# menyifang/MIMO

Measured on NVIDIA H100. Metric: frames/sec @ 512x512x24f, 20 DDIM steps, higher is better.
Workload: dtype fp16

## Files before the change

include/mimo_b200.h:

```cpp
#ifndef MIMO_B200_H_
#define MIMO_B200_H_

#include <stdint.h>

#ifdef __cplusplus
extern "C" {
#endif

#define MIMO_OK 0
#define MIMO_ERR_ARG (-1)
#define MIMO_ERR_CUDA (-2)
#define MIMO_ERR_DEVICE (-3)

#define MIMO_F16 0
#define MIMO_BF16 1

#define MIMO_ACT_NONE 0
#define MIMO_ACT_SILU 1
#define MIMO_ACT_GEGLU 2

const char* mimo_version(void);
const char* mimo_last_error(void);
int mimo_device_check(int dev);
int mimo_abi_sizeof(int which);

typedef struct {
  const void* bias;
  const void* rowvec;
  int64_t rows_per_group;
  int64_t ld_rowvec;
  const void* residual;
  int64_t ld_res;
  float scale;
  int act;
} mimo_epilogue;

typedef struct {
  const void* a;
  int64_t lda;
  const void* a1;
  int64_t lda1;
  const void* w;
  int64_t ldw;
  void* out;
  int64_t ldo;
  int32_t M, N, K;
  int32_t K1;
  int32_t dtype;
  mimo_epilogue ep;
  void* workspace;
  int64_t workspace_bytes;
} mimo_gemm_params;
int mimo_gemm(const mimo_gemm_params* p, void* stream);
int mimo_gemm_geglu_granule(int32_t N);

typedef struct {
  const void* a;
  int64_t lda;
  const float* a_scale;
  const void* w;
  int64_t ldw;
  const float* w_scale;
  void* out;
  int64_t ldo;
  int32_t M, N, K;
  int32_t dtype;
  mimo_epilogue ep;
  void* workspace;
  int64_t workspace_bytes;
} mimo_gemm_e4m3_params;
int mimo_gemm_e4m3(const mimo_gemm_e4m3_params* p, void* stream);

typedef struct {
  const void* x0;
  int32_t c0;
  const void* x1;
  int32_t c1;
  const void* w;
  void* out;
  int64_t ldo;
  int32_t n, h, w_, cout;
  int32_t dtype;
  mimo_epilogue ep;
  void* workspace;
  int64_t workspace_bytes;
} mimo_conv3x3_params;
int mimo_conv3x3(const mimo_conv3x3_params* p, void* stream);
int mimo_conv_up2x(const mimo_conv3x3_params* p, void* stream);

int mimo_im2col3x3(const void* x, void* col, int32_t n, int32_t h, int32_t w, int32_t c, int32_t stride,
                   int32_t upshift, int32_t pad_lo, int64_t ldcol, int32_t dtype, void* stream);

typedef struct {
  const void* x0;
  int32_t c0;
  const void* x1;
  int32_t c1;
  const void* gamma;
  const void* beta;
  void* out;
  float* stats;
  int32_t n, hw, groups;
  float eps;
  int32_t silu;
  int32_t dtype;
} mimo_groupnorm_params;
int mimo_groupnorm(const mimo_groupnorm_params* p, void* stream);
int64_t mimo_groupnorm_workspace_bytes(const mimo_groupnorm_params* p);

typedef struct {
  const void* x0;
  int32_t c0;
  const void* x1;
  int32_t c1;
  const void* gamma;
  const void* beta;
  void* out;
  float* table;
  int64_t table_bytes;
  float* stats;
  int32_t samples, frames, table_frames, hw, groups;
  float eps;
  int32_t silu;
  int32_t dtype;
} mimo_groupnorm_window_params;
int mimo_groupnorm_window(const mimo_groupnorm_window_params* p, void* stream);
int mimo_groupnorm_window_partials(const mimo_groupnorm_window_params* p, void* stream);
int mimo_groupnorm_window_apply(const mimo_groupnorm_window_params* p, void* stream);
int64_t mimo_groupnorm_window_table_bytes(const mimo_groupnorm_window_params* p);

int mimo_layernorm(const void* x, const void* gamma, const void* beta, void* out, int64_t rows, int32_t c,
                   float eps, const void* pe, int64_t rows_per_frame, int32_t frames, int32_t pe_frame_offset,
                   int32_t dtype, void* stream);
int mimo_layernorm_e4m3(const void* x, const void* gamma, const void* beta, void* out, float* scale, int64_t rows,
                        int32_t c, float eps, const void* pe, int64_t rows_per_frame, int32_t frames,
                        int32_t pe_frame_offset, int32_t dtype, void* stream);

typedef struct {
  const void* q;
  const void* k;
  const void* v;
  int64_t ld_qkv;
  const void* bank_k;
  const void* bank_v;
  int64_t ld_bank;
  int32_t lb;
  int32_t nb;
  const int32_t* bank_index;
  void* out;
  int64_t ld_out;
  int32_t n, lq, heads, d;
  float scale;
  int32_t dtype;
} mimo_attn_params;
int mimo_attn_spatial(const mimo_attn_params* p, void* stream);

typedef struct {
  const void* q;
  int64_t ld_q;
  const void* k;
  const void* v;
  int64_t ld_kv;
  void* out;
  int64_t ld_out;
  int64_t chunk_stride_rows;
  int32_t batch, q_frames, kv_frames, frames_per_chunk;
  int32_t hw, heads, d;
  float scale;
  int32_t dtype;
} mimo_attn_temporal_params;
int mimo_attn_temporal(const mimo_attn_temporal_params* p, void* stream);

#define MIMO_MAX_PEERS 8
typedef struct {
  const void* peer_src[MIMO_MAX_PEERS];
  void* peer_ready[MIMO_MAX_PEERS];
  void* ctl;
  void* dst;
  const void* residual;
  int32_t mode, G, r;
  int32_t b, fl, hw, C;
  int32_t dtype;
  int32_t max_blocks;
  int32_t timeout_ms;
} mimo_exchange_params;
int mimo_exchange(const mimo_exchange_params* p, void* stream);
int mimo_peer_alloc(int64_t bytes, void** ptr, void* handle64);
int mimo_peer_open(const void* handle64, void** ptr);
int mimo_peer_close(void* ptr);
int mimo_peer_free(void* ptr);

int mimo_ncfhw_to_nhwc(const void* src, void* dst, int32_t b, int32_t c, int32_t f, int32_t h, int32_t w,
                       int32_t cpad, int32_t src_is_f32, int32_t dtype, void* stream);
int mimo_nhwc_to_ncfhw(const void* src, void* dst, int32_t b, int32_t c, int32_t f, int32_t h, int32_t w,
                       int32_t ld, int32_t dst_is_f32, int32_t dtype, void* stream);
int mimo_upsample2x(const void* x, void* out, int32_t n, int32_t h, int32_t w, int32_t c, int32_t dtype, void* stream);
int mimo_upsample_nearest(const void* x, void* out, int32_t n, int32_t h, int32_t w, int32_t oh, int32_t ow, int32_t c,
                          int32_t dtype, void* stream);
int mimo_softmax_rows(void* x, int64_t rows, int32_t cols, int64_t ld, int32_t dtype, void* stream);
int mimo_add(const void* a, const void* b, void* out, int64_t count, int32_t dtype, void* stream);
int mimo_silu(const void* x, void* out, int64_t count, int32_t dtype, void* stream);

int mimo_quick_gelu(const void* x, void* out, int64_t count, int32_t dtype, void* stream);

int mimo_composite_frame(const void* canvas, const void* bk, const float* mask, const void* occ, const void* vid,
                         const void* prev, double factor, void* out, int64_t pixels, void* stream);
// ... 36 lines not shown
```

mimo_b200/csrc/gemm_wgmma.cu:

```cuda
#include <cuda_runtime.h>

#include <cudaTypedefs.h>

#include "../../include/mimo_b200.h"
#include "host_util.h"
#include "ptx.cuh"
#include "wgmma.cuh"

namespace mimo {

constexpr int BM = 128;
constexpr int BK = 64;
constexpr int kGemmThreads = 320;
constexpr int kChunk = 8192;

struct EpiArgs {
  const void* bias;
  const void* rowvec;
  long long rows_per_group;
  long long ld_rowvec;
  float scale;
  int act;
  float* partial;
};

struct ConvGeom {
  int conv;
  int H, W, NI;
  int TW, TH, TN;
  int tiles_w, tiles_h;
  int ctot;
  int c0;
  int kb0, kb1;
  int a_bytes;
  int chunk_bytes;
  int splits;
  int kb_split;
  int ntaps;
  signed char tdx[9], tdy[9];
};

template <int BN, bool kRes, bool kE4m3 = false>
struct GemmCfg {
  static constexpr int kStageBytes = BM * BK * 2 + BN * BK * 2;
  static constexpr int kNChunk = BN / 32;
  static constexpr int kOutBytes = 2 * kChunk;
  static constexpr int kResSlots = kRes ? 2 : 0;
  static constexpr int kResBytes = kResSlots * kChunk;
  static constexpr int kBarBytes = 512;
  static constexpr int kFixed = kBarBytes + 2048  + (kE4m3 ? 3072  : 0) + kOutBytes + kResBytes;
  static constexpr int kMaxStages = (BN >= 256) ? 4 : (BN >= 160 ? 5 : (BN >= 128 ? 6 : 8));
  static constexpr int kFit = (227 * 1024 - kFixed) / kStageBytes;
  static constexpr int kStages = kFit < kMaxStages ? kFit : kMaxStages;
  static constexpr int kSmemBytes = kStages * kStageBytes + kFixed;
  static_assert(kStages >= 3, "pipeline too shallow");
};

template <int BN, bool kBf16, bool kRes>
__global__ void __launch_bounds__(kGemmThreads, 1)
gemm_wgmma_kernel(const __grid_constant__ CUtensorMap tmA0, const __grid_constant__ CUtensorMap tmA1,
                  const __grid_constant__ CUtensorMap tmB, const __grid_constant__ CUtensorMap tmOut,
                  const __grid_constant__ CUtensorMap tmRes, int M, int N, int num_m_tiles, int num_n_tiles,
                  int num_k_blocks, ConvGeom g, EpiArgs ep) {
  constexpr bool kE4m3 = false;
  constexpr const float* a_scale = nullptr;
  constexpr const float* w_scale = nullptr;
#include "gemm_wgmma_body.cuh"
}

template <int BN, bool kBf16, bool kRes>
__global__ void __launch_bounds__(kGemmThreads, 1)
gemm_e4m3_kernel(const __grid_constant__ CUtensorMap tmA0, const __grid_constant__ CUtensorMap tmA1,
                 const __grid_constant__ CUtensorMap tmB, const __grid_constant__ CUtensorMap tmOut,
                 const __grid_constant__ CUtensorMap tmRes, int M, int N, int num_m_tiles, int num_n_tiles,
                 int num_k_blocks, ConvGeom g, EpiArgs ep, const float* __restrict__ a_scale,
                 const float* __restrict__ w_scale) {
  constexpr bool kE4m3 = true;
#include "gemm_wgmma_body.cuh"
}


template <bool kBf16>
__global__ void __launch_bounds__(256)
splitk_reduce_kernel(const float* __restrict__ part, int splits, long long M, int N, const void* __restrict__ bias,
                     const void* __restrict__ rowvec, long long rpg, long long ld_rowvec,
                     const void* __restrict__ res, long long ld_res, float scale, int act, void* __restrict__ out,
                     long long ldo) {
  using C = Cvt<kBf16>;
  using T = typename C::T;
  pdl_launch_dependents();
  pdl_wait();
  const int nv = N >> 3;
  const long long idx = blockIdx.x * static_cast<long long>(blockDim.x) + threadIdx.x;
  if (idx >= M * nv) return;
  const long long row = idx / nv;
  const int col = static_cast<int>(idx - row * nv) * 8;
  float a[8] = {0.f, 0.f, 0.f, 0.f, 0.f, 0.f, 0.f, 0.f};
  for (int s = 0; s < splits; ++s) {
    const float4* p = reinterpret_cast<const float4*>(part + (static_cast<long long>(s) * M + row) * N + col);
    const float4 u0 = p[0], u1 = p[1];
    a[0] += u0.x, a[1] += u0.y, a[2] += u0.z, a[3] += u0.w;
    a[4] += u1.x, a[5] += u1.y, a[6] += u1.z, a[7] += u1.w;
  }
  float cst[8] = {0.f, 0.f, 0.f, 0.f, 0.f, 0.f, 0.f, 0.f};
  auto add_vec = [&](const T* v, float* dst, bool scaled_fma) {
    const uint4 b = *reinterpret_cast<const uint4*>(v);
    const uint32_t w[4] = {b.x, b.y, b.z, b.w};
#pragma unroll
    for (int j = 0; j < 4; ++j) {
      const float2 t = C::unpack(w[j]);
      if (scaled_fma) {
        dst[2 * j] = fmaf(t.x, scale, dst[2 * j]);
        dst[2 * j + 1] = fmaf(t.y, scale, dst[2 * j + 1]);
      } else {
        dst[2 * j] += t.x;
        dst[2 * j + 1] += t.y;
      }
    }
  };
  if (bias) add_vec(static_cast<const T*>(bias) + col, cst, false);
  if (rowvec) add_vec(static_cast<const T*>(rowvec) + (row / rpg) * ld_rowvec + col, cst, false);
  float f[8];
#pragma unroll
  for (int j = 0; j < 8; ++j) f[j] = fmaf(a[j], scale, cst[j] * scale);
  if (res) add_vec(static_cast<const T*>(res) + row * ld_res + col, f, true);
  if (act == MIMO_ACT_SILU) {
#pragma unroll
    for (int j = 0; j < 8; ++j) f[j] = silu_f(f[j]);
  }
  uint4 o;
  o.x = C::pack(f[0], f[1]);
  o.y = C::pack(f[2], f[3]);
  o.z = C::pack(f[4], f[5]);
  o.w = C::pack(f[6], f[7]);
  *reinterpret_cast<uint4*>(static_cast<T*>(out) + row * ldo + col) = o;
}

static int pick_splits(long long tiles, int nkb, long long M, int N, int64_t ws_bytes) {
  if (tiles * 2 > num_sms() || nkb < 32) return 1;
  long long s = num_sms() / tiles;
  if (s > nkb / 16) s = nkb / 16;
  if (s > 16) s = 16;
  while (s > 1 && s * M * N * 4 > ws_bytes) --s;
  return s < 2 ? 1 : static_cast<int>(s);
}

struct Maps {
  CUtensorMap a0, a1, b, out, res;
};

template <int BN, bool kBf16, bool kRes>
static int launch_cfg(const Maps& m, int M, int N, int mt, int nt, int nkb, const ConvGeom& g, const EpiArgs& ep,
                      cudaStream_t st) {
  using Cfg = GemmCfg<BN, kRes>;
  auto kern = gemm_wgmma_kernel<BN, kBf16, kRes>;
  static bool attr_done = false;
  if (!attr_done) {
    cudaError_t e = cudaFuncSetAttribute(kern, cudaFuncAttributeMaxDynamicSharedMemorySize, Cfg::kSmemBytes);
    if (e != cudaSuccess) return set_cuda_error("cudaFuncSetAttribute(gemm)", e);
    attr_done = true;
  }
  const int tiles = mt * nt;
  const int grid = tiles < num_sms() ? tiles : num_sms();
  cudaError_t e = launch_k(kern, dim3(grid), dim3(kGemmThreads), Cfg::kSmemBytes, st, m.a0, m.a1, m.b, m.out, m.res, M, N, mt,
                           nt, nkb, g, ep);
  if (e == cudaSuccess) e = cudaGetLastError();
  if (e != cudaSuccess) return set_cuda_error("gemm launch", e);
  return MIMO_OK;
}

template <bool kBf16>
static int launch_bn(int bn, bool res, const Maps& m, int M, int N, int mt, int nt, int nkb, const ConvGeom& g,
                     const EpiArgs& ep, cudaStream_t st) {
  switch (bn) {
    case 64:
      return res ? launch_cfg<64, kBf16, true>(m, M, N, mt, nt, nkb, g, ep, st)
                 : launch_cfg<64, kBf16, false>(m, M, N, mt, nt, nkb, g, ep, st);
    case 128:
      return res ? launch_cfg<128, kBf16, true>(m, M, N, mt, nt, nkb, g, ep, st)
                 : launch_cfg<128, kBf16, false>(m, M, N, mt, nt, nkb, g, ep, st);
    case 160:
      return res ? launch_cfg<160, kBf16, true>(m, M, N, mt, nt, nkb, g, ep, st)
                 : launch_cfg<160, kBf16, false>(m, M, N, mt, nt, nkb, g, ep, st);
    case 192:
      return res ? launch_cfg<192, kBf16, true>(m, M, N, mt, nt, nkb, g, ep, st)
                 : launch_cfg<192, kBf16, false>(m, M, N, mt, nt, nkb, g, ep, st);
    case 256:
      return res ? launch_cfg<256, kBf16, true>(m, M, N, mt, nt, nkb, g, ep, st)
                 : launch_cfg<256, kBf16, false>(m, M, N, mt, nt, nkb, g, ep, st);
  }
  return set_error(MIMO_ERR_ARG, "gemm: unsupported BN");
}

int pick_bn(int N, bool geglu, long long m_tiles);

template <bool kBf16>
static int launch_e4m3(int bn, bool res, const Maps& m, int M, int N, int mt, int nt, int nkb, const ConvGeom& g,
                       const EpiArgs& ep, const float* a_scale, const float* w_scale, cudaStream_t st) {
  auto run = [&](auto kern, int smem) -> int {
    static bool attr_done[2][2][2] = {};
    bool& done = attr_done[bn == 256][kBf16][res];
    if (!done) {
      cudaError_t e = cudaFuncSetAttribute(kern, cudaFuncAttributeMaxDynamicSharedMemorySize, smem);
      if (e != cudaSuccess) return set_cuda_error("cudaFuncSetAttribute(gemm_e4m3)", e);
      done = true;
    }
    const int tiles = mt * nt;
    const int grid = tiles < num_sms() ? tiles : num_sms();
    cudaError_t e = launch_k(kern, dim3(grid), dim3(kGemmThreads), smem, st, m.a0, m.a1, m.b, m.out, m.res, M, N, mt, nt,
                             nkb, g, ep, a_scale, w_scale);
    if (e == cudaSuccess) e = cudaGetLastError();
    if (e != cudaSuccess) return set_cuda_error("gemm_e4m3 launch", e);
    return MIMO_OK;
  };
  if (bn == 192)
    return res ? run(gemm_e4m3_kernel<192, kBf16, true>, GemmCfg<192, true, true>::kSmemBytes)
               : run(gemm_e4m3_kernel<192, kBf16, false>, GemmCfg<192, false, true>::kSmemBytes);
  if (bn == 256)
    return res ? run(gemm_e4m3_kernel<256, kBf16, true>, GemmCfg<256, true, true>::kSmemBytes)
               : run(gemm_e4m3_kernel<256, kBf16, false>, GemmCfg<256, false, true>::kSmemBytes);
  return set_error(MIMO_ERR_ARG, "mimo_gemm_e4m3: unsupported BN");
}

static int pick_bn_e4m3(int N, bool geglu) {
  if (geglu) return pick_bn(N, true, 1 << 20);
  const int pad256 = (N + 255) / 256 * 256 - N, pad192 = (N + 191) / 192 * 192 - N;
  return pad192 < pad256 ? 192 : 256;
}

static int g_force_bn = 0;

int pick_bn(int N, bool geglu, long long m_tiles) {
  if (g_force_bn) return g_force_bn;
  if (geglu) {
    if (N % 256 == 0) return 256;
    if (N % 128 == 0) return 128;
    return 64;
  }
  const int cands[5] = {256, 192, 160, 128, 64};
  int best = 64;
  double best_eff = -1.0;
  for (int i = 0; i < 5; ++i) {
    const int bn = cands[i];
    const int nt = (N + bn - 1) / bn;
    double eff = static_cast<double>(N) / (static_cast<double>(nt) * bn);
    const long long tiles = m_tiles * nt;
    if (tiles < num_sms() && bn > 64) eff *= 0.5 + 0.5 * static_cast<double>(tiles) / num_sms();
    if (eff > best_eff + 1e-9) {
      best_eff = eff;
      best = bn;
    }
  }
  return best;
}

static EpiArgs make_epi(const mimo_epilogue& e, int N) {
  EpiArgs a;
  a.bias = e.bias;
  a.rowvec = e.rowvec;
  a.rows_per_group = e.rows_per_group > 0 ? e.rows_per_group : 1;
  if (a.rows_per_group > 0x7fffffffLL) a.rows_per_group = 0x7fffffffLL;
  a.ld_rowvec = e.ld_rowvec > 0 ? e.ld_rowvec : N;
  a.scale = e.scale;
  a.act = e.act;
  a.partial = nullptr;
  return a;
}

static int g_splitk = 0;

static int launch_reduce(int dtype, const float* part, int splits, long long M, int N, const mimo_epilogue& e, void* out,
                         long long ldo, cudaStream_t st) {
  const long long total = M * (N / 8);
  const unsigned blocks = div_up(total, 256);
  const long long rpg = e.rows_per_group > 0 ? e.rows_per_group : 1;
  const long long ldr = e.ld_rowvec > 0 ? e.ld_rowvec : N;
  cudaError_t err = dtype == MIMO_BF16
                        ? launch_k(splitk_reduce_kernel<true>, dim3(blocks), dim3(256), 0, st, part, splits, M, N, e.bias,
                                   e.rowvec, rpg, ldr, e.residual, static_cast<long long>(e.ld_res), e.scale, e.act, out, ldo)
                        : launch_k(splitk_reduce_kernel<false>, dim3(blocks), dim3(256), 0, st, part, splits, M, N, e.bias,
                                   e.rowvec, rpg, ldr, e.residual, static_cast<long long>(e.ld_res), e.scale, e.act, out, ldo);
  if (err == cudaSuccess) err = cudaGetLastError();
  if (err != cudaSuccess) return set_cuda_error("split-K reduce launch", err);
  return MIMO_OK;
}

}

using namespace mimo;

extern "C" int mimo_debug_splitk(int mode) {
  g_splitk = mode;
  return 0;
}

extern "C" int mimo_debug_force_bn(int bn) {
  g_force_bn = bn;
  return 0;
}

extern "C" int mimo_gemm_geglu_granule(int32_t N) { return pick_bn(N, true, 1 << 20) / 2; }

extern "C" int mimo_gemm(const mimo_gemm_params* p, void* stream) {
  if (!p || !p->a || !p->w || !p->out) return set_error(MIMO_ERR_ARG, "mimo_gemm: null pointer");
  if (p->M <= 0 || p->N <= 0 || p->K <= 0) return set_error(MIMO_ERR_ARG, "mimo_gemm: empty problem");
  if ((p->K % 8) || (p->lda % 8) || (p->ldw % 8) || (p->N % 8) || (p->ldo % 8))
    return set_error(MIMO_ERR_ARG, "mimo_gemm: K, N, lda, ldw, ldo must be multiples of 8");
  if (p->ep.residual && (p->ep.ld_res % 8)) return set_error(MIMO_ERR_ARG, "mimo_gemm: ld_res % 8 != 0");
  const bool geglu = p->ep.act == MIMO_ACT_GEGLU;
  if (geglu && (p->ep.residual || p->ep.rowvec))
    return set_error(MIMO_ERR_ARG, "mimo_gemm: GEGLU takes neither a residual nor a row vector");
  if (int rc = ensure_device()) return rc;
  const int mt = (p->M + BM - 1) / BM;
  const int K1 = p->a1 ? p->K1 : 0;
  if (K1 < 0 || (K1 % 8) || (p->a1 && (p->lda1 % 8))) return set_error(MIMO_ERR_ARG, "mimo_gemm: K1/lda1 % 8 != 0");
  const int kb0 = (p->K + BK - 1) / BK;
  const int kb1 = (K1 + BK - 1) / BK;
  const int nkb = kb0 + kb1;
  int bn = pick_bn(p->N, geglu, mt);
  int splits = 1;
  if (!geglu && g_splitk && p->workspace && !g_force_bn) {
    const int bn_wide = pick_bn(p->N, false, 1 << 20);
    splits = pick_splits(static_cast<long long>(mt) * ((p->N + bn_wide - 1) / bn_wide), nkb, p->M, p->N, p->workspace_bytes);
    if (splits > 1) bn = bn_wide;
  }
  if (geglu && (p->N % bn)) return set_error(MIMO_ERR_ARG, "mimo_gemm: GEGLU needs N % tile == 0");
  const int nt = (p->N + bn - 1) / bn;
  const bool res = p->ep.residual != nullptr && !geglu && splits == 1;

  Maps m;
  const uint64_t adim[2] = {static_cast<uint64_t>(p->K), static_cast<uint64_t>(p->M)};
  const uint64_t astr[1] = {static_cast<uint64_t>(p->lda) * 2};
  const uint32_t abox[2] = {BK, BM};
  if (int rc = encode_tmap(&m.a0, p->dtype, 2, p->a, adim, astr, abox)) return rc;
  m.a1 = m.a0;
  if (K1) {
    const uint64_t a1dim[2] = {static_cast<uint64_t>(K1), static_cast<uint64_t>(p->M)};
    const uint64_t a1str[1] = {static_cast<uint64_t>(p->lda1) * 2};
    if (int rc = encode_tmap(&m.a1, p->dtype, 2, p->a1, a1dim, a1str, abox)) return rc;
  }
  const uint64_t bdim[2] = {static_cast<uint64_t>(p->K + K1), static_cast<uint64_t>(p->N)};
  const uint64_t bstr[1] = {static_cast<uint64_t>(p->ldw) * 2};
  const uint32_t bbox[2] = {BK, static_cast<uint32_t>(bn)};
  if (int rc = encode_tmap(&m.b, p->dtype, 2, p->w, bdim, bstr, bbox)) return rc;
  const int n_out = geglu ? p->N / 2 : p->N;
  const uint64_t odim[2] = {static_cast<uint64_t>(n_out), static_cast<uint64_t>(p->M)};
  const uint64_t ostr[1] = {static_cast<uint64_t>(p->ldo) * 2};
  const uint32_t obox[2] = {32, BM};
  if (int rc = encode_tmap(&m.out, p->dtype, 2, p->out, odim, ostr, obox, 64)) return rc;
  m.res = m.out;
  if (res) {
    const uint64_t rstr[1] = {static_cast<uint64_t>(p->ep.ld_res) * 2};
    if (int rc = encode_tmap(&m.res, p->dtype, 2, p->ep.residual, odim, rstr, obox, 64)) return rc;
  }

  ConvGeom g = {};
  g.kb0 = kb0;
  g.kb1 = kb1;
  g.c0 = p->K;
  g.chunk_bytes = kChunk;
  g.splits = splits;
  g.kb_split = (nkb + splits - 1) / splits;
  EpiArgs ep = make_epi(p->ep, p->N);
  cudaStream_t st = static_cast<cudaStream_t>(stream);
  if (splits > 1) {
    ep.bias = ep.rowvec = nullptr;
    ep.act = MIMO_ACT_NONE;
    ep.scale = 1.0f;
    ep.partial = static_cast<float*>(p->workspace);
  }
  const int rc = p->dtype == MIMO_BF16 ? launch_bn<true>(bn, res, m, p->M, p->N, mt, nt, nkb, g, ep, st)
                                       : launch_bn<false>(bn, res, m, p->M, p->N, mt, nt, nkb, g, ep, st);
  if (rc || splits == 1) return rc;
  return launch_reduce(p->dtype, ep.partial, splits, p->M, p->N, p->ep, p->out, p->ldo, st);
}

extern "C" int mimo_gemm_e4m3(const mimo_gemm_e4m3_params* p, void* stream) {
  if (!p || !p->a || !p->w || !p->out || !p->a_scale || !p->w_scale)
    return set_error(MIMO_ERR_ARG, "mimo_gemm_e4m3: null pointer");
  if (p->M <= 0 || p->N <= 0 || p->K <= 0) return set_error(MIMO_ERR_ARG, "mimo_gemm_e4m3: empty problem");
  if ((p->K % 16) || (p->lda % 16) || (p->ldw % 16))
    return set_error(MIMO_ERR_ARG, "mimo_gemm_e4m3: K, lda, ldw must be multiples of 16");
  if ((p->N % 8) || (p->ldo % 8)) return set_error(MIMO_ERR_ARG, "mimo_gemm_e4m3: N, ldo must be multiples of 8");
  if ((reinterpret_cast<uintptr_t>(p->a) | reinterpret_cast<uintptr_t>(p->w) | reinterpret_cast<uintptr_t>(p->out) |
       reinterpret_cast<uintptr_t>(p->ep.residual)) % 16)
    return set_error(MIMO_ERR_ARG, "mimo_gemm_e4m3: a, w, out, residual must be 16-byte aligned");
  if (p->ep.residual && (p->ep.ld_res % 8)) return set_error(MIMO_ERR_ARG, "mimo_gemm_e4m3: ld_res % 8 != 0");
  if (p->workspace || p->workspace_bytes) return set_error(MIMO_ERR_ARG, "mimo_gemm_e4m3: split-K is not supported");
  const bool geglu = p->ep.act == MIMO_ACT_GEGLU;
  if (geglu && (p->ep.residual || p->ep.rowvec))
    return set_error(MIMO_ERR_ARG, "mimo_gemm_e4m3: GEGLU takes neither a residual nor a row vector");
  const int bn = pick_bn_e4m3(p->N, geglu);
  if (geglu && (p->N % bn)) return set_error(MIMO_ERR_ARG, "mimo_gemm_e4m3: GEGLU needs N % tile == 0");
  if (bn != 192 && bn != 256) return set_error(MIMO_ERR_ARG, "mimo_gemm_e4m3: GEGLU needs N % 256 == 0");
  if (int rc = ensure_device()) return rc;
  const int mt = (p->M + BM - 1) / BM;
  const int nt = (p->N + bn - 1) / bn;
  const int nkb = (p->K + 2 * BK - 1) / (2 * BK);
  const bool res = p->ep.residual != nullptr && !geglu;

  Maps m;
  const uint64_t adim[2] = {static_cast<uint64_t>(p->K), static_cast<uint64_t>(p->M)};
  const uint64_t astr[1] = {static_cast<uint64_t>(p->lda)};
  const uint32_t abox[2] = {2 * BK, BM};
  if (int rc = encode_tmap(&m.a0, kTmapU8, 2, p->a, adim, astr, abox)) return rc;
  m.a1 = m.a0;
  const uint64_t bdim[2] = {static_cast<uint64_t>(p->K), static_cast<uint64_t>(p->N)};
  const uint64_t bstr[1] = {static_cast<uint64_t>(p->ldw)};
  const uint32_t bbox[2] = {2 * BK, static_cast<uint32_t>(bn)};
  if (int rc = encode_tmap(&m.b, kTmapU8, 2, p->w, bdim, bstr, bbox)) return rc;
  const int n_out = geglu ? p->N / 2 : p->N;
  const uint64_t odim[2] = {static_cast<uint64_t>(n_out), static_cast<uint64_t>(p->M)};
  const uint64_t ostr[1] = {static_cast<uint64_t>(p->ldo) * 2};
  const uint32_t obox[2] = {32, BM};
  if (int rc = encode_tmap(&m.out, p->dtype, 2, p->out, odim, ostr, obox, 64)) return rc;
  m.res = m.out;
  if (res) {
    const uint64_t rstr[1] = {static_cast<uint64_t>(p->ep.ld_res) * 2};
    if (int rc = encode_tmap(&m.res, p->dtype, 2, p->ep.residual, odim, rstr, obox, 64)) return rc;
  }
  ConvGeom g = {};
  g.kb0 = nkb;
  g.c0 = p->K;
  g.chunk_bytes = kChunk;
  g.splits = 1;
  g.kb_split = nkb;
  const EpiArgs ep = make_epi(p->ep, p->N);
  cudaStream_t st = static_cast<cudaStream_t>(stream);
  return p->dtype == MIMO_BF16 ? launch_e4m3<true>(bn, res, m, p->M, p->N, mt, nt, nkb, g, ep, p->a_scale, p->w_scale, st)
                               : launch_e4m3<false>(bn, res, m, p->M, p->N, mt, nt, nkb, g, ep, p->a_scale, p->w_scale, st);
}

static int conv_launch(const mimo_conv3x3_params* p, const void* w, int ntaps, const signed char* tdx,
                       const signed char* tdy, void* out, int sx, int sy, int ow, int oh, void* stream) {
  const int c1 = p->x1 ? p->c1 : 0;
  ConvGeom g = {};
  g.conv = 1;
  g.H = p->h;
  g.W = p->w_;
  g.NI = p->n;
  g.TW = p->w_ < BM ? p->w_ : BM;
  g.TH = BM / g.TW;
  if (g.TH > p->h) g.TH = p->h;
  if (g.TH < 1) g.TH = 1;
  g.TN = BM / (g.TW * g.TH);
  if (g.TN > p->n) g.TN = p->n;
  if (g.TN < 1) g.TN = 1;
  if (g.TN > 1 && g.TH != p->h) g.TN = 1;
  g.tiles_w = (p->w_ + g.TW - 1) / g.TW;
  g.tiles_h = (p->h + g.TH - 1) / g.TH;
  const int tiles_n = (p->n + g.TN - 1) / g.TN;
  g.ctot = p->c0 + c1;
  g.c0 = p->c0;
  g.kb0 = (p->c0 + BK - 1) / BK;
  g.kb1 = (c1 + BK - 1) / BK;
  g.a_bytes = g.TW * g.TH * g.TN * BK * 2;
  g.chunk_bytes = g.TW * g.TH * g.TN * 64;
  g.ntaps = ntaps;
  for (int t = 0; t < 9; ++t) {
    g.tdx[t] = t < ntaps ? tdx[t] : 0;
    g.tdy[t] = t < ntaps ? tdy[t] : 0;
  }
  const int mt = g.tiles_w * g.tiles_h * tiles_n;
  const int nkb = ntaps * (g.kb0 + g.kb1);
  const long long Mrows = static_cast<long long>(p->n) * p->h * p->w_;
  if (Mrows > 0x7fffffffLL) return set_error(MIMO_ERR_ARG, "mimo_conv: too many pixels");
  int bn = pick_bn(p->cout, false, mt);
  int splits = 1;
  if (g_splitk && p->workspace && !g_force_bn && sx == 1 && sy == 1 && p->ldo == p->cout) {
    const int bn_wide = pick_bn(p->cout, false, 1 << 20);
    splits = pick_splits(static_cast<long long>(mt) * ((p->cout + bn_wide - 1) / bn_wide), nkb, Mrows, p->cout,
                         p->workspace_bytes);
    if (splits > 1) bn = bn_wide;
  }
  g.splits = splits;
  g.kb_split = (nkb + splits - 1) / splits;
  const int nt = (p->cout + bn - 1) / bn;
  const bool res = p->ep.residual != nullptr && splits == 1;

  Maps m;
  auto nhwc_map = [&](CUtensorMap* tm, const void* base, int c, long long pitch, uint32_t box_c, int swz, int px,
                      int py, int iw, int ih) {
    const uint64_t dim[4] = {static_cast<uint64_t>(c), static_cast<uint64_t>(p->w_), static_cast<uint64_t>(p->h),
                             static_cast<uint64_t>(p->n)};
    const uint64_t str[3] = {static_cast<uint64_t>(px) * pitch * 2, static_cast<uint64_t>(py) * iw * pitch * 2,
                             static_cast<uint64_t>(ih) * iw * pitch * 2};
    const uint32_t box[4] = {box_c, static_cast<uint32_t>(g.TW), static_cast<uint32_t>(g.TH),
                             static_cast<uint32_t>(g.TN)};
    return encode_tmap(tm, p->dtype, 4, base, dim, str, box, swz);
  };
  if (int rc = nhwc_map(&m.a0, p->x0, p->c0, p->c0, BK, 128, 1, 1, p->w_, p->h)) return rc;
  m.a1 = m.a0;
  if (c1)
    if (int rc = nhwc_map(&m.a1, p->x1, c1, c1, BK, 128, 1, 1, p->w_, p->h)) return rc;
  {
    const uint64_t dim[2] = {static_cast<uint64_t>(ntaps) * g.ctot, static_cast<uint64_t>(p->cout)};
    const uint64_t str[1] = {static_cast<uint64_t>(ntaps) * g.ctot * 2};
    const uint32_t box[2] = {BK, static_cast<uint32_t>(bn)};
    if (int rc = encode_tmap(&m.b, p->dtype, 2, w, dim, str, box)) return rc;
  }
  if (int rc = nhwc_map(&m.out, out, p->cout, p->ldo, 32, 64, sx, sy, ow, oh)) return rc;
  m.res = m.out;
  if (res)
    if (int rc = nhwc_map(&m.res, p->ep.residual, p->cout, p->ep.ld_res, 32, 64, 1, 1, p->w_, p->h)) return rc;

  EpiArgs ep = make_epi(p->ep, p->cout);
  cudaStream_t st = static_cast<cudaStream_t>(stream);
  if (splits > 1) {
    ep.bias = ep.rowvec = nullptr;
    ep.act = MIMO_ACT_NONE;
    ep.scale = 1.0f;
    ep.partial = static_cast<float*>(p->workspace);
  }
  const int rc = p->dtype == MIMO_BF16
                     ? launch_bn<true>(bn, res, m, static_cast<int>(Mrows), p->cout, mt, nt, nkb, g, ep, st)
                     : launch_bn<false>(bn, res, m, static_cast<int>(Mrows), p->cout, mt, nt, nkb, g, ep, st);
  if (rc || splits == 1) return rc;
// ... 41 lines not shown
```

mimo_b200/lib.py:

```python
from __future__ import annotations

import ctypes as C
import os
from pathlib import Path

_PKG = Path(__file__).resolve().parent
LIB_PATH = _PKG / "libmimo_b200.so"

F16, BF16 = 0, 1
ACT_NONE, ACT_SILU, ACT_GEGLU = 0, 1, 2


class MimoError(RuntimeError):
    pass


class Epilogue(C.Structure):
    _fields_ = [
        ("bias", C.c_void_p),
        ("rowvec", C.c_void_p),
        ("rows_per_group", C.c_int64),
        ("ld_rowvec", C.c_int64),
        ("residual", C.c_void_p),
        ("ld_res", C.c_int64),
        ("scale", C.c_float),
        ("act", C.c_int),
    ]


class GemmParams(C.Structure):
    _fields_ = [
        ("a", C.c_void_p), ("lda", C.c_int64),
        ("a1", C.c_void_p), ("lda1", C.c_int64),
        ("w", C.c_void_p), ("ldw", C.c_int64),
        ("out", C.c_void_p), ("ldo", C.c_int64),
        ("M", C.c_int32), ("N", C.c_int32), ("K", C.c_int32), ("K1", C.c_int32),
        ("dtype", C.c_int32),
        ("ep", Epilogue),
        ("workspace", C.c_void_p), ("workspace_bytes", C.c_int64),
    ]


class GemmE4m3Params(C.Structure):
    _fields_ = [
        ("a", C.c_void_p), ("lda", C.c_int64), ("a_scale", C.c_void_p),
        ("w", C.c_void_p), ("ldw", C.c_int64), ("w_scale", C.c_void_p),
        ("out", C.c_void_p), ("ldo", C.c_int64),
        ("M", C.c_int32), ("N", C.c_int32), ("K", C.c_int32),
        ("dtype", C.c_int32),
        ("ep", Epilogue),
        ("workspace", C.c_void_p), ("workspace_bytes", C.c_int64),
    ]


class Conv3x3Params(C.Structure):
    _fields_ = [
        ("x0", C.c_void_p), ("c0", C.c_int32),
        ("x1", C.c_void_p), ("c1", C.c_int32),
        ("w", C.c_void_p),
        ("out", C.c_void_p), ("ldo", C.c_int64),
        ("n", C.c_int32), ("h", C.c_int32), ("w_", C.c_int32), ("cout", C.c_int32),
        ("dtype", C.c_int32),
        ("ep", Epilogue),
        ("workspace", C.c_void_p), ("workspace_bytes", C.c_int64),
    ]


class GroupNormParams(C.Structure):
    _fields_ = [
        ("x0", C.c_void_p), ("c0", C.c_int32),
        ("x1", C.c_void_p), ("c1", C.c_int32),
        ("gamma", C.c_void_p), ("beta", C.c_void_p),
        ("out", C.c_void_p),
        ("stats", C.c_void_p),
        ("n", C.c_int32), ("hw", C.c_int32), ("groups", C.c_int32),
        ("eps", C.c_float),
        ("silu", C.c_int32),
        ("dtype", C.c_int32),
    ]


class GroupNormWindowParams(C.Structure):
    _fields_ = [
        ("x0", C.c_void_p), ("c0", C.c_int32),
        ("x1", C.c_void_p), ("c1", C.c_int32),
        ("gamma", C.c_void_p), ("beta", C.c_void_p),
        ("out", C.c_void_p),
        ("table", C.c_void_p), ("table_bytes", C.c_int64),
        ("stats", C.c_void_p),
        ("samples", C.c_int32), ("frames", C.c_int32), ("table_frames", C.c_int32), ("hw", C.c_int32),
        ("groups", C.c_int32),
        ("eps", C.c_float),
        ("silu", C.c_int32),
        ("dtype", C.c_int32),
    ]


class AttnParams(C.Structure):
    _fields_ = [
        ("q", C.c_void_p), ("k", C.c_void_p), ("v", C.c_void_p), ("ld_qkv", C.c_int64),
        ("bank_k", C.c_void_p), ("bank_v", C.c_void_p), ("ld_bank", C.c_int64),
        ("lb", C.c_int32), ("nb", C.c_int32),
        ("bank_index", C.c_void_p),
        ("out", C.c_void_p), ("ld_out", C.c_int64),
        ("n", C.c_int32), ("lq", C.c_int32), ("heads", C.c_int32), ("d", C.c_int32),
        ("scale", C.c_float),
        ("dtype", C.c_int32),
    ]


class AttnTemporalParams(C.Structure):
    _fields_ = [
        ("q", C.c_void_p), ("ld_q", C.c_int64),
        ("k", C.c_void_p), ("v", C.c_void_p), ("ld_kv", C.c_int64),
        ("out", C.c_void_p), ("ld_out", C.c_int64),
        ("chunk_stride_rows", C.c_int64),
        ("batch", C.c_int32), ("q_frames", C.c_int32), ("kv_frames", C.c_int32), ("frames_per_chunk", C.c_int32),
        ("hw", C.c_int32), ("heads", C.c_int32), ("d", C.c_int32),
        ("scale", C.c_float),
        ("dtype", C.c_int32),
    ]


MAX_PEERS = 8


class ExchangeParams(C.Structure):
    _fields_ = [
        ("peer_src", C.c_void_p * MAX_PEERS), ("peer_ready", C.c_void_p * MAX_PEERS),
        ("ctl", C.c_void_p), ("dst", C.c_void_p), ("residual", C.c_void_p),
        ("mode", C.c_int32), ("G", C.c_int32), ("r", C.c_int32),
        ("b", C.c_int32), ("fl", C.c_int32), ("hw", C.c_int32), ("C", C.c_int32),
        ("dtype", C.c_int32), ("max_blocks", C.c_int32), ("timeout_ms", C.c_int32),
    ]


class CfgMultistepParams(C.Structure):
    _fields_ = [
        ("pred_uncond", C.c_void_p), ("pred_cond", C.c_void_p), ("counter", C.c_void_p), ("frame_stride", C.c_int64),
        ("latents", C.c_void_p), ("count", C.c_int64),
        ("hist_out", C.c_void_p), ("h1", C.c_void_p), ("h2", C.c_void_p), ("noise", C.c_void_p),
        ("guidance", C.c_float), ("a", C.c_float), ("b", C.c_float),
        ("c_x", C.c_float), ("c_m", C.c_float), ("c_1", C.c_float), ("c_2", C.c_float), ("c_n", C.c_float),
        ("dtype", C.c_int32),
    ]


_VP, _I32, _I64, _F = C.c_void_p, C.c_int32, C.c_int64, C.c_float
SYMBOLS = {
    "mimo_version": (C.c_char_p, []),
    "mimo_last_error": (C.c_char_p, []),
    "mimo_device_check": (C.c_int, [C.c_int]),
    "mimo_abi_sizeof": (C.c_int, [C.c_int]),
    "mimo_gemm": (C.c_int, [C.POINTER(GemmParams), _VP]),
    "mimo_gemm_geglu_granule": (C.c_int, [_I32]),
    "mimo_gemm_e4m3": (C.c_int, [C.POINTER(GemmE4m3Params), _VP]),
    "mimo_conv3x3": (C.c_int, [C.POINTER(Conv3x3Params), _VP]),
    "mimo_conv_up2x": (C.c_int, [C.POINTER(Conv3x3Params), _VP]),
    "mimo_im2col3x3": (C.c_int, [_VP, _VP, _I32, _I32, _I32, _I32, _I32, _I32, _I32, _I64, _I32, _VP]),
    "mimo_groupnorm": (C.c_int, [C.POINTER(GroupNormParams), _VP]),
    "mimo_groupnorm_workspace_bytes": (C.c_int64, [C.POINTER(GroupNormParams)]),
    "mimo_groupnorm_window": (C.c_int, [C.POINTER(GroupNormWindowParams), _VP]),
    "mimo_groupnorm_window_partials": (C.c_int, [C.POINTER(GroupNormWindowParams), _VP]),
    "mimo_groupnorm_window_apply": (C.c_int, [C.POINTER(GroupNormWindowParams), _VP]),
    "mimo_groupnorm_window_table_bytes": (C.c_int64, [C.POINTER(GroupNormWindowParams)]),
    "mimo_layernorm": (C.c_int, [_VP, _VP, _VP, _VP, _I64, _I32, _F, _VP, _I64, _I32, _I32, _I32, _VP]),
    "mimo_layernorm_e4m3": (C.c_int, [_VP, _VP, _VP, _VP, _VP, _I64, _I32, _F, _VP, _I64, _I32, _I32, _I32, _VP]),
    "mimo_attn_spatial": (C.c_int, [C.POINTER(AttnParams), _VP]),
    "mimo_attn_temporal": (C.c_int, [C.POINTER(AttnTemporalParams), _VP]),
    "mimo_exchange": (C.c_int, [C.POINTER(ExchangeParams), _VP]),
    "mimo_peer_alloc": (C.c_int, [_I64, C.POINTER(C.c_void_p), C.c_char_p]),
    "mimo_peer_open": (C.c_int, [C.c_char_p, C.POINTER(C.c_void_p)]),
    "mimo_peer_close": (C.c_int, [_VP]),
    "mimo_peer_free": (C.c_int, [_VP]),
    "mimo_ncfhw_to_nhwc": (C.c_int, [_VP, _VP, _I32, _I32, _I32, _I32, _I32, _I32, _I32, _I32, _VP]),
    "mimo_nhwc_to_ncfhw": (C.c_int, [_VP, _VP, _I32, _I32, _I32, _I32, _I32, _I32, _I32, _I32, _VP]),
    "mimo_upsample2x": (C.c_int, [_VP, _VP, _I32, _I32, _I32, _I32, _I32, _VP]),
    "mimo_upsample_nearest": (C.c_int, [_VP, _VP, _I32, _I32, _I32, _I32, _I32, _I32, _I32, _VP]),
    "mimo_softmax_rows": (C.c_int, [_VP, _I64, _I32, _I64, _I32, _VP]),
    "mimo_add": (C.c_int, [_VP, _VP, _VP, _I64, _I32, _VP]),
    "mimo_silu": (C.c_int, [_VP, _VP, _I64, _I32, _VP]),
    "mimo_quick_gelu": (C.c_int, [_VP, _VP, _I64, _I32, _VP]),
    "mimo_composite_frame": (C.c_int, [_VP, _VP, _VP, _VP, _VP, _VP, C.c_double, _VP, _I64, _VP]),
    "mimo_cfg_ddim_step": (C.c_int, [_VP, _VP, _VP, _I64, _VP, _I64, _F, _F, _F, _F, _F, _I32, _VP]),
    "mimo_cfg_ddim_step_noise": (C.c_int, [_VP, _VP, _VP, _I64, _VP, _I64, _F, _F, _F, _F, _F, _VP, _F, _I32, _VP]),
    "mimo_interpolate_frames": (C.c_int, [_VP, _VP, _I32, _I64, _I32, _I32, _I32, _VP]),
    "mimo_cfg_multistep": (C.c_int, [C.POINTER(CfgMultistepParams), _VP]),
}
_DEBUG_SYMBOLS = {"mimo_debug_pdl": (C.c_int, [C.c_int]), "mimo_debug_splitk": (C.c_int, [C.c_int]),
                  "mimo_debug_force_bn": (C.c_int, [C.c_int])}

_lib = None


def load() -> C.CDLL:
    global _lib
    if _lib is not None:
        return _lib
    if not LIB_PATH.exists():
        raise MimoError(
            f"{LIB_PATH} is missing: run `python -m mimo_b200.build` (or __graft_entry__.build()). "
            "mimo_b200 has no CPU or PyTorch fallback."
        )
    lib = C.CDLL(os.fspath(LIB_PATH))
    for name, (res, args) in {**SYMBOLS, **_DEBUG_SYMBOLS}.items():
        fn = getattr(lib, name)
        fn.restype = res
        fn.argtypes = args
    for which, st in enumerate((Epilogue, GemmParams, Conv3x3Params, GroupNormParams, AttnParams, AttnTemporalParams,
                             ExchangeParams, CfgMultistepParams, GroupNormWindowParams, GemmE4m3Params)):
        if lib.mimo_abi_sizeof(which) != C.sizeof(st):
            raise MimoError(f"ABI mismatch: {st.__name__} is {C.sizeof(st)} bytes in lib.py but "
                            f"{lib.mimo_abi_sizeof(which)} in {LIB_PATH.name}; rebuild the library")
    if os.environ.get("MIMO_B200_PDL") in ("0", "1"):
        lib.mimo_debug_pdl(int(os.environ["MIMO_B200_PDL"]))
    _lib = lib
    return lib


def check(rc: int, what: str = "") -> None:
    if rc != 0:
        msg = load().mimo_last_error().decode(errors="replace")
        raise MimoError(f"{what or 'mimo call'} failed (rc={rc}): {msg}")
```

Baseline: 8.057.

## Add warp-specialized persistent GEMM with SMEM-resident weight panel for small K

Adds a persistent, warp-specialized WGMMA GEMM kernel for problems with at most five K-blocks. Each CTA keeps the whole B (weight) panel for one N tile resident in shared memory and streams 64-row A tiles through a deep TMA ring. Two consumer warpgroups alternate M tiles so one tile's epilogue can overlap the other's MMA, with separate producer warps for A and residual loads. The path is chosen automatically when there are enough M tiles per CTA, and a debug switch can turn it off or force it. It adds a sizeable new kernel with intricate barrier logic and less reuse of A in exchange for not reloading weights per tile.

```diff
diff --git a/include/mimo_b200.h b/include/mimo_b200.h
--- a/include/mimo_b200.h
+++ b/include/mimo_b200.h
@@ -52,6 +52,7 @@
   int64_t workspace_bytes;
 } mimo_gemm_params;
 int mimo_gemm(const mimo_gemm_params* p, void* stream);
+int mimo_debug_gemm_ws(int mode);
 int mimo_gemm_geglu_granule(int32_t N);
 
 typedef struct {
diff --git a/mimo_b200/csrc/gemm_wgmma.cu b/mimo_b200/csrc/gemm_wgmma.cu
--- a/mimo_b200/csrc/gemm_wgmma.cu
+++ b/mimo_b200/csrc/gemm_wgmma.cu
@@ -78,6 +78,8 @@
   constexpr bool kE4m3 = true;
 #include "gemm_wgmma_body.cuh"
 }
+
+#include "gemm_ws.cuh"
 
 
 template <bool kBf16>
@@ -269,6 +271,40 @@
 
 static int g_splitk = 0;
 
+static int g_gemm_ws = 0;
+constexpr int kWsMinTilesPerCta = 8;
+
+static bool ws_instantiated(int bn, bool res) { return bn == 160 || (!res && (bn == 192 || bn == 256)); }
+
+template <int BN, bool kBf16, bool kRes>
+static int launch_ws_cfg(const Maps& m, int M, int N, int mt, int nkb, int groups, int group_ctas, const EpiArgs& ep,
+                         cudaStream_t st) {
+  using Cfg = WsCfg<BN, kRes>;
+  auto kern = gemm_ws_kernel<BN, kBf16, kRes>;
+  static bool attr_done = false;
+  if (!attr_done) {
+    cudaError_t e = cudaFuncSetAttribute(kern, cudaFuncAttributeMaxDynamicSharedMemorySize, Cfg::kSmemBytes);
+    if (e != cudaSuccess) return set_cuda_error("cudaFuncSetAttribute(gemm_ws)", e);
+    attr_done = true;
+  }
+  cudaError_t e = launch_k(kern, dim3(groups * group_ctas), dim3(kGemmThreads), Cfg::kSmemBytes, st, m.a0, m.b, m.out,
+                           m.res, M, N, mt, nkb, groups, group_ctas, ep);
+  if (e == cudaSuccess) e = cudaGetLastError();
+  if (e != cudaSuccess) return set_cuda_error("gemm_ws launch", e);
+  return MIMO_OK;
+}
+
+template <bool kBf16>
+static int launch_ws(int bn, bool res, const Maps& m, int M, int N, int mt, int nkb, int groups, int group_ctas,
+                     const EpiArgs& ep, cudaStream_t st) {
+  if (bn == 160)
+    return res ? launch_ws_cfg<160, kBf16, true>(m, M, N, mt, nkb, groups, group_ctas, ep, st)
+               : launch_ws_cfg<160, kBf16, false>(m, M, N, mt, nkb, groups, group_ctas, ep, st);
+  if (bn == 192 && !res) return launch_ws_cfg<192, kBf16, false>(m, M, N, mt, nkb, groups, group_ctas, ep, st);
+  if (bn == 256 && !res) return launch_ws_cfg<256, kBf16, false>(m, M, N, mt, nkb, groups, group_ctas, ep, st);
+  return set_error(MIMO_ERR_ARG, "gemm_ws: unsupported BN");
+}
+
 static int launch_reduce(int dtype, const float* part, int splits, long long M, int N, const mimo_epilogue& e, void* out,
                          long long ldo, cudaStream_t st) {
   const long long total = M * (N / 8);
@@ -297,6 +333,12 @@
 extern "C" int mimo_debug_force_bn(int bn) {
   g_force_bn = bn;
   return 0;
+}
+
+extern "C" int mimo_debug_gemm_ws(int mode) {
+  if (mode < 0 || mode > 2) return set_error(MIMO_ERR_ARG, "mimo_debug_gemm_ws: mode must be 0 (auto), 1 (off) or 2 (force)");
+  g_gemm_ws = mode;
+  return MIMO_OK;
 }
 
 extern "C" int mimo_gemm_geglu_granule(int32_t N) { return pick_bn(N, true, 1 << 20) / 2; }
@@ -328,10 +370,19 @@
   const int nt = (p->N + bn - 1) / bn;
   const bool res = p->ep.residual != nullptr && !geglu && splits == 1;
 
+  const int mt64 = (p->M + kWsBM - 1) / kWsBM;
+  const int ws_ctas = nt < num_sms() ? nt : num_sms();
+  int ws_groups = num_sms() / ws_ctas;
+  if (g_gemm_ws == 2 && ws_groups > mt64 / 2) ws_groups = mt64 / 2;
+  const bool ws = g_gemm_ws != 1 && splits == 1 && !K1 && nkb <= kWsMaxKb && ws_instantiated(bn, res) &&
+                  ws_groups >= 1 &&
+                  (g_gemm_ws == 2 || mt64 >= static_cast<long long>(kWsMinTilesPerCta) * ws_groups);
+
   Maps m;
   const uint64_t adim[2] = {static_cast<uint64_t>(p->K), static_cast<uint64_t>(p->M)};
   const uint64_t astr[1] = {static_cast<uint64_t>(p->lda) * 2};
-  const uint32_t abox[2] = {BK, BM};
+  const uint32_t box_rows = ws ? kWsBM : BM;
+  const uint32_t abox[2] = {BK, box_rows};
   if (int rc = encode_tmap(&m.a0, p->dtype, 2, p->a, adim, astr, abox)) return rc;
   m.a1 = m.a0;
   if (K1) {
@@ -346,12 +397,18 @@
   const int n_out = geglu ? p->N / 2 : p->N;
   const uint64_t odim[2] = {static_cast<uint64_t>(n_out), static_cast<uint64_t>(p->M)};
   const uint64_t ostr[1] = {static_cast<uint64_t>(p->ldo) * 2};
-  const uint32_t obox[2] = {32, BM};
+  const uint32_t obox[2] = {32, box_rows};
   if (int rc = encode_tmap(&m.out, p->dtype, 2, p->out, odim, ostr, obox, 64)) return rc;
   m.res = m.out;
   if (res) {
     const uint64_t rstr[1] = {static_cast<uint64_t>(p->ep.ld_res) * 2};
     if (int rc = encode_tmap(&m.res, p->dtype, 2, p->ep.residual, odim, rstr, obox, 64)) return rc;
+  }
+  cudaStream_t st = static_cast<cudaStream_t>(stream);
+  if (ws) {
+    const EpiArgs ep = make_epi(p->ep, p->N);
+    return p->dtype == MIMO_BF16 ? launch_ws<true>(bn, res, m, p->M, p->N, mt64, nkb, ws_groups, ws_ctas, ep, st)
+                                 : launch_ws<false>(bn, res, m, p->M, p->N, mt64, nkb, ws_groups, ws_ctas, ep, st);
   }
 
   ConvGeom g = {};
@@ -362,7 +419,6 @@
   g.splits = splits;
   g.kb_split = (nkb + splits - 1) / splits;
   EpiArgs ep = make_epi(p->ep, p->N);
-  cudaStream_t st = static_cast<cudaStream_t>(stream);
   if (splits > 1) {
     ep.bias = ep.rowvec = nullptr;
     ep.act = MIMO_ACT_NONE;
diff --git a/mimo_b200/csrc/gemm_ws.cuh b/mimo_b200/csrc/gemm_ws.cuh
--- /dev/null
+++ b/mimo_b200/csrc/gemm_ws.cuh
@@ -0,0 +1,319 @@
+
+constexpr int kWsMaxKb = 5;
+constexpr int kWsBM = 64;
+constexpr int kWsChunk = kWsBM * 64;
+constexpr int kWsMaxStages = 12;
+
+template <int BN, bool kRes>
+struct WsCfg {
+  static constexpr int kPanelBytes = kWsMaxKb * BN * BK * 2;
+  static constexpr int kStageBytes = kWsBM * BK * 2;
+  static constexpr int kNChunk = BN / 32;
+  static constexpr int kOutBytes = 2 * 2 * kWsChunk;
+  static constexpr int kResBytes = kRes ? 2 * kNChunk * kWsChunk : 0;
+  static constexpr int kConstBytes = 2 * 256 * 4;
+  static constexpr int kBarBytes = 512;
+  static constexpr int kFixed = kPanelBytes + kOutBytes + kResBytes + kConstBytes + kBarBytes;
+  static constexpr int kFit = (227 * 1024 - kFixed) / kStageBytes;
+  static constexpr int kStages = kFit < kWsMaxStages ? kFit : kWsMaxStages;
+  static constexpr int kSmemBytes = kFixed + kStages * kStageBytes;
+  static_assert(kStages >= 4, "A ring too shallow");
+};
+
+template <int BN, bool kBf16, bool kRes>
+__global__ void __launch_bounds__(kGemmThreads, 1)
+gemm_ws_kernel(const __grid_constant__ CUtensorMap tmA, const __grid_constant__ CUtensorMap tmB,
+               const __grid_constant__ CUtensorMap tmOut, const __grid_constant__ CUtensorMap tmRes, int M, int N,
+               int num_m_tiles, int num_k_blocks, int groups, int group_ctas, EpiArgs ep) {
+  using Cfg = WsCfg<BN, kRes>;
+  using C = Cvt<kBf16>;
+  using T = typename C::T;
+  constexpr int NCHUNK = Cfg::kNChunk;
+  constexpr int S = Cfg::kStages;
+  extern __shared__ __align__(1024) uint8_t smem[];
+  uint8_t* sPanel = smem;
+  uint8_t* sA = sPanel + Cfg::kPanelBytes;
+  uint8_t* sOutAll = sA + S * Cfg::kStageBytes;
+  uint8_t* sResAll = sOutAll + Cfg::kOutBytes;
+  float* sConstAll = reinterpret_cast<float*>(sResAll + Cfg::kResBytes);
+  uint64_t* bars = reinterpret_cast<uint64_t*>(reinterpret_cast<uint8_t*>(sConstAll) + Cfg::kConstBytes);
+  uint64_t* full_bar = bars;
+  uint64_t* empty_bar = bars + kWsMaxStages;
+  uint64_t* res_full = bars + 2 * kWsMaxStages;
+  uint64_t* res_empty = res_full + 2;
+  uint64_t* panel_full = res_empty + 2;
+  uint64_t* panel_empty = panel_full + 1;
+
+  pdl_launch_dependents();
+  const int warp = __shfl_sync(0xffffffffu, threadIdx.x >> 5, 0);
+  const int lane = threadIdx.x & 31;
+  const int P = group_ctas;
+  const int grp = blockIdx.x / P;
+  const int n0 = blockIdx.x - grp * P;
+  const int m_begin = static_cast<int>(static_cast<long long>(num_m_tiles) * grp / groups);
+  const int L = static_cast<int>(static_cast<long long>(num_m_tiles) * (grp + 1) / groups) - m_begin;
+  const int num_n_tiles = (N + BN - 1) / BN;
+  const int nseg = (num_n_tiles - n0 + P - 1) / P;
+  const int total = nseg * L;
+  const int nkb = num_k_blocks;
+
+  if (warp == 8 && lane == 0) {
+    tma_prefetch_desc(&tmA);
+    tma_prefetch_desc(&tmB);
+    tma_prefetch_desc(&tmOut);
+    if (kRes) tma_prefetch_desc(&tmRes);
+  }
+  if (warp == 9 && lane == 0) {
+    for (int s = 0; s < S; ++s) {
+      mbar_init(&full_bar[s], 1);
+      mbar_init(&empty_bar[s], 4);
+    }
+    for (int w = 0; w < 2; ++w) {
+      mbar_init(&res_full[w], 1);
+      mbar_init(&res_empty[w], 4);
+    }
+    mbar_init(panel_full, 1);
+    mbar_init(panel_empty, 8);
+    fence_mbar_init();
+  }
+  __syncthreads();
+  pdl_wait();
+
+  if (warp == 8) {
+    uint32_t stage = 0, phase = 0;
+    for (int seg = 0; seg < nseg; ++seg) {
+      const int n_tile = n0 + seg * P;
+      if (seg > 0) mbar_wait(panel_empty, (seg - 1) & 1);
+      if (elect_one()) {
+        mbar_expect_tx(panel_full, nkb * BN * BK * 2);
+        for (int kb = 0; kb < nkb; ++kb)
+          tma_load_2d(sPanel + kb * BN * BK * 2, &tmB, panel_full, kb * BK, n_tile * BN);
+      }
+      __syncwarp();
+      for (int i = 0; i < L; ++i) {
+        for (int kb = 0; kb < nkb; ++kb) {
+          mbar_wait(&empty_bar[stage], phase ^ 1u);
+          if (elect_one()) {
+            mbar_expect_tx(&full_bar[stage], Cfg::kStageBytes);
+            tma_load_2d(sA + stage * Cfg::kStageBytes, &tmA, &full_bar[stage], kb * BK, (m_begin + i) * kWsBM);
+          }
+          __syncwarp();
+          if (++stage == S) {
+            stage = 0;
+            phase ^= 1u;
+          }
+        }
+      }
+    }
+  } else if (warp == 9) {
+    if constexpr (kRes) {
+      int seg = 0, i = 0;
+      for (int j = 0; j < total; ++j) {
+        const int w = j & 1;
+        mbar_wait(&res_empty[w], ((j >> 1) & 1) ^ 1u);
+        if (elect_one()) {
+          mbar_expect_tx(&res_full[w], NCHUNK * kWsChunk);
+          for (int c = 0; c < NCHUNK; ++c)
+            tma_load_2d(sResAll + (w * NCHUNK + c) * kWsChunk, &tmRes, &res_full[w], (n0 + seg * P) * BN + c * 32,
+                        (m_begin + i) * kWsBM);
+        }
+        __syncwarp();
+        if (++i == L) {
+          i = 0;
+          ++seg;
+        }
+      }
+    }
+  } else if (warp < 8) {
+    const int wg = warp >> 2;
+    const int ct = threadIdx.x & 127;
+    const int rbase = (warp & 3) * 16 + (lane >> 2);
+    const int q2 = (lane & 3) * 2;
+    const bool issuer = ct == 0;
+    const int sw[2] = {(rbase >> 1) & 3, ((rbase + 8) >> 1) & 3};
+    const bool do_silu = ep.act == MIMO_ACT_SILU;
+    const uint32_t rpg = static_cast<uint32_t>(ep.rows_per_group);
+    uint8_t* sOut = sOutAll + wg * 2 * kWsChunk;
+    [[maybe_unused]] uint8_t* sRes = sResAll + wg * NCHUNK * kWsChunk;
+    float* sb = sConstAll + wg * 256;
+    const int bar_epi = 1 + wg, bar_mine = 3 + wg, bar_other = 4 - wg;
+    float acc[BN / 2];
+    uint32_t stage = 0, phase = 0, oc = 0;
+    auto skip_tile = [&]() {
+      for (int s = 0; s < nkb; ++s)
+        if (++stage == S) {
+          stage = 0;
+          phase ^= 1u;
+        }
+    };
+    if (wg == 1) skip_tile();
+    int seg = 0, i = wg, seg_ready = -1;
+
+    for (int j = wg; j < total; j += 2) {
+      const int m_tile = m_begin + i, n_tile = n0 + seg * P;
+      if (seg != seg_ready) {
+        mbar_wait(panel_full, seg & 1);
+        seg_ready = seg;
+      }
+      auto block_groups = [&](uint32_t& gf, uint32_t& gl) {
+        const uint32_t m0 = static_cast<uint32_t>(m_tile >> 1) * 128u;
+        uint32_t m1 = m0 + 127u;
+        if (m1 > static_cast<uint32_t>(M) - 1) m1 = static_cast<uint32_t>(M) - 1;
+        gf = m0 / rpg;
+        gl = m1 / rpg;
+      };
+      auto load_consts = [&](int ce) -> float {
+        float v = 0.f;
+        const int col = n_tile * BN + ce;
+        if (col < N) {
+          if (ep.bias) v = C::to_f(static_cast<const T*>(ep.bias)[col]);
+          if (ep.rowvec) {
+            uint32_t gf, gl;
+            block_groups(gf, gl);
+            if (gf == gl) v += C::to_f(static_cast<const T*>(ep.rowvec)[static_cast<long long>(gf) * ep.ld_rowvec + col]);
+          }
+        }
+        return ep.act == MIMO_ACT_GEGLU ? v : v * ep.scale;
+      };
+      if (ct < BN) sb[ct] = load_consts(ct);
+      if (ct + 128 < BN) sb[ct + 128] = load_consts(ct + 128);
+
+      if (j > 0) bar_sync(bar_mine, 256);
+      uint32_t prev_stage = 0;
+      for (int kb = 0; kb < nkb; ++kb) {
+        mbar_wait(&full_bar[stage], phase);
+        const uint64_t da = make_smem_desc_sw128(smem_u32(sA + stage * Cfg::kStageBytes), 16, 1024);
+        const uint64_t db = make_smem_desc_sw128(smem_u32(sPanel + kb * BN * BK * 2), 16, 1024);
+        wgmma_fence();
+#pragma unroll
+        for (int k = 0; k < BK / 16; ++k) Wgmma<BN, kBf16>::ss(acc, da + 2 * k, db + 2 * k, (kb | k) != 0 ? 1u : 0u);
+        wgmma_commit();
+        if (kb > 0) {
+          wgmma_wait<1>();
+          if (lane == 0) mbar_arrive(&empty_bar[prev_stage]);
+        }
+        prev_stage = stage;
+        if (++stage == S) {
+          stage = 0;
+          phase ^= 1u;
+        }
+      }
+      if (j + 1 < total) bar_arrive(bar_other, 256);
+      wgmma_wait<0>();
+      reg_fence(acc);
+      if (lane == 0) mbar_arrive(&empty_bar[prev_stage]);
+      skip_tile();
+      int next_i = i + 2, next_seg = seg;
+      while (next_i >= L) {
+        next_i -= L;
+        ++next_seg;
+      }
+      if (next_seg != seg && lane == 0) mbar_arrive(panel_empty);
+
+      long long row[2];
+      bool row_ok[2];
+#pragma unroll
+      for (int h = 0; h < 2; ++h) {
+        row[h] = static_cast<long long>(m_tile) * kWsBM + rbase + 8 * h;
+        row_ok[h] = row[h] < M;
+      }
+      bar_sync(bar_epi, 128);
+      if constexpr (kRes) mbar_wait(&res_full[wg], (j >> 1) & 1);
+
+      auto stage_and_store = [&](uint8_t* obuf, int col0) {
+        fence_proxy_async_smem();
+        if (issuer) tma_store_wait_read0();
+        bar_sync(bar_epi, 128);
+        if (issuer) {
+          tma_store_2d(&tmOut, obuf, col0, m_tile * kWsBM);
+          tma_store_commit();
+        }
+      };
+
+      if (ep.act != MIMO_ACT_GEGLU) {
+        const float scale = ep.scale;
+        bool rv_uniform = false;
+        if (ep.rowvec) {
+          uint32_t gf, gl;
+          block_groups(gf, gl);
+          rv_uniform = gf == gl;
+        }
+        const bool need_rv = ep.rowvec != nullptr && !rv_uniform;
+        const int mode = (!kRes && !do_silu && !need_rv && ep.bias == nullptr && ep.rowvec == nullptr && scale == 1.0f)
+                             ? 0 : (need_rv ? 2 : 1);
+        const T* rv[2];
+#pragma unroll
+        for (int h = 0; h < 2; ++h)
+          rv[h] = (need_rv && row_ok[h])
+                      ? static_cast<const T*>(ep.rowvec) + static_cast<long long>(static_cast<uint32_t>(row[h]) / rpg) * ep.ld_rowvec
+                      : nullptr;
+#pragma unroll
+        for (int c = 0; c < NCHUNK; ++c) {
+          uint8_t* obuf = sOut + (oc & 1u) * kWsChunk;
+          ++oc;
+          const int col0 = n_tile * BN + c * 32;
+#pragma unroll
+          for (int jj = 0; jj < 4; ++jj) {
+            const int jf = 4 * c + jj;
+            const float2 cst0 = *reinterpret_cast<const float2*>(sb + c * 32 + 8 * jj + q2);
+#pragma unroll
+            for (int h = 0; h < 2; ++h) {
+              const int r = rbase + 8 * h;
+              const int off = r * 64 + ((jj ^ sw[h]) << 4) + q2 * 2;
+              float f0 = acc[4 * jf + 2 * h], f1 = acc[4 * jf + 2 * h + 1];
+              if (mode != 0) {
+                float c0 = cst0.x, c1 = cst0.y;
+                if (mode == 2 && rv[h] && col0 + 8 * jj + q2 < N) {
+                  const float2 t = C::unpack(__ldg(reinterpret_cast<const unsigned int*>(rv[h] + col0 + 8 * jj + q2)));
+                  c0 = fmaf(t.x, scale, c0);
+                  c1 = fmaf(t.y, scale, c1);
+                }
+                f0 = fmaf(f0, scale, c0);
+                f1 = fmaf(f1, scale, c1);
+              }
+              if constexpr (kRes) {
+                const float2 t = C::unpack(*reinterpret_cast<const uint32_t*>(sRes + c * kWsChunk + off));
+                f0 = fmaf(t.x, scale, f0);
+                f1 = fmaf(t.y, scale, f1);
+              }
+              if (do_silu) {
+                f0 = silu_f(f0);
+                f1 = silu_f(f1);
+              }
+              *reinterpret_cast<uint32_t*>(obuf + off) = C::pack(f0, f1);
+            }
+          }
+          stage_and_store(obuf, col0);
+        }
+        if constexpr (kRes) {
+          __syncwarp();
+          if (lane == 0) mbar_arrive(&res_empty[wg]);
+        }
+      } else {
+        constexpr int HALF = BN / 2;
+#pragma unroll
+        for (int c = 0; c < HALF / 32; ++c) {
+          uint8_t* obuf = sOut + (oc & 1u) * kWsChunk;
+          ++oc;
+#pragma unroll
+          for (int jj = 0; jj < 4; ++jj) {
+            const int jf = 4 * c + jj, jg = jf + HALF / 8;
+            const float2 cv = *reinterpret_cast<const float2*>(sb + c * 32 + 8 * jj + q2);
+            const float2 cg = *reinterpret_cast<const float2*>(sb + HALF + c * 32 + 8 * jj + q2);
+#pragma unroll
+            for (int h = 0; h < 2; ++h) {
+              const int r = rbase + 8 * h;
+              const float f0 = (acc[4 * jf + 2 * h] + cv.x) * gelu_erf_fast(acc[4 * jg + 2 * h] + cg.x);
+              const float f1 = (acc[4 * jf + 2 * h + 1] + cv.y) * gelu_erf_fast(acc[4 * jg + 2 * h + 1] + cg.y);
+              *reinterpret_cast<uint32_t*>(obuf + r * 64 + ((jj ^ sw[h]) << 4) + q2 * 2) = C::pack(f0, f1);
+            }
+          }
+          stage_and_store(obuf, n_tile * HALF + c * 32);
+        }
+      }
+      i = next_i;
+      seg = next_seg;
+    }
+    if (issuer) tma_store_wait_all();
+  }
+}
diff --git a/mimo_b200/lib.py b/mimo_b200/lib.py
--- a/mimo_b200/lib.py
+++ b/mimo_b200/lib.py
@@ -154,6 +154,7 @@
     "mimo_abi_sizeof": (C.c_int, [C.c_int]),
     "mimo_gemm": (C.c_int, [C.POINTER(GemmParams), _VP]),
     "mimo_gemm_geglu_granule": (C.c_int, [_I32]),
+    "mimo_debug_gemm_ws": (C.c_int, [C.c_int]),
     "mimo_gemm_e4m3": (C.c_int, [C.POINTER(GemmE4m3Params), _VP]),
     "mimo_conv3x3": (C.c_int, [C.POINTER(Conv3x3Params), _VP]),
     "mimo_conv_up2x": (C.c_int, [C.POINTER(Conv3x3Params), _VP]),
```

Measured after the change: 8.244 (median of 6 runs). 1.02x the previous value.
